# Autobot37/weatherforecastingtoolkit

Measured on AMD Instinct MI355X. Metric: SEVIR 384x384 frames/sec (AE train step), higher is better.
Workload: dtype f32; 1 GPU; experiments/ae_v2 conv AE (ae_64x8x8_lin.PosAwareAE_TF, img_size=384), 1x384x384 synthetic SEVIR frames, batch 32/GPU, fp32, fwd + L1 + bwd + AdamW + cosine-warmup LR; batch_per_gpu=32, global_batch=32, img_size=384, parallelism=dp1, params=215033281

## Files before the change

### include/wfae.h

```cpp
#ifndef WFAE_H
#define WFAE_H

#include <stddef.h>
#include <stdint.h>

#ifdef __cplusplus
extern "C" {
#endif

typedef void* wfae_stream_t;

typedef enum {
  WFAE_OK = 0,
  WFAE_ERR_BAD_SHAPE = -1,
  WFAE_ERR_NULL_POINTER = -2,
  WFAE_ERR_WORKSPACE = -3,
  WFAE_ERR_LAUNCH = -4,
  WFAE_ERR_UNSUPPORTED = -5
} wfae_status;

int wfae_version(void);
const char* wfae_last_error_string(void);
size_t wfae_workspace_bytes(int64_t max_weight_elems);

enum { WFAE_PRECISION_FP32 = 0, WFAE_PRECISION_BF16 = 1 };
int wfae_set_matmul_precision(int mode);
int wfae_get_matmul_precision(void);

int wfae_set_split_gemm(int on);
int wfae_get_split_gemm(void);

int wfae_set_c1n(int on);
int wfae_get_c1n(void);

int wfae_conv1x1_fwd(const float* x, const float* w, const float* bias, const float* res,
                     int64_t res_img_stride, float* y, int NB, int Cin, int Cout, int HW,
                     wfae_stream_t stream);
int wfae_conv1x1_fwd_stats(const float* x, const float* w, const float* bias, const float* res,
                           int64_t res_img_stride, float* y, int NB, int Cin, int Cout, int HW,
                           double* stat_part, int64_t stat_capacity, int* stat_rows, wfae_stream_t stream);
int wfae_conv1x1_fwd_bnact(const float* x, const float* bn_scale, const float* bn_shift, const float* w,
                           const float* bias, const float* res, int64_t res_img_stride, float* y, int NB, int Cin,
                           int Cout, int HW, double* stat_part, int64_t stat_capacity, int* stat_rows,
                           wfae_stream_t stream);
int wfae_conv1x1_bwd_weight_bnact(const float* dy, const float* x, const float* bn_scale, const float* bn_shift,
                                  float* dw, int NB, int Cin, int Cout, int HW, int accumulate, void* ws,
                                  size_t ws_bytes, wfae_stream_t stream);
int wfae_conv1x1_bwd_data(const float* dy, const float* w, float* dx, int NB, int Cin, int Cout,
                          int HW, wfae_stream_t stream);
int wfae_conv1x1_bwd_weight(const float* dy, const float* x, float* dw, int NB, int Cin, int Cout,
                            int HW, int accumulate, void* ws, size_t ws_bytes, wfae_stream_t stream);

int wfae_c1r_supported(int M, int K, int HW);
int wfae_c1r_stat_rows(int M, int K, int NB, int HW);
int wfae_c1r_fwd(const float* w, int64_t w_sm, int64_t w_sk, const float* x, const float* pro_scale, const float* pro_shift,
                 const float* res, float* y, int NB, int K, int M, int HW, double* stat_part, int64_t stat_capacity,
                 int* stat_rows, wfae_stream_t stream);
int wfae_c1r_bnred_supported(int M, int K, int HW);
int wfae_c1r_bnred(const float* w, int64_t w_sm, int64_t w_sk, const float* dt, const float* x, const float* bn_scale,
                   const float* bn_shift, const float* save_mean, const float* save_invstd, float* da, int NB, int K, int M, int HW,
                   double* part, int64_t part_capacity, int* part_rows, wfae_stream_t stream);
int wfae_bn_act_bwd_from_rows(const double* part, int rows, int C, float* dgamma, float* dbeta, int accumulate, void* ws,
                              size_t ws_bytes, wfae_stream_t stream);
int wfae_c1r_bndx(const float* w, int64_t w_sm, int64_t w_sk, const float* dt, const float* x, const float* gamma,
                  const float* bn_scale, const float* bn_shift, const float* save_mean, const float* save_invstd, const float* coef,
                  const float* res, float* dx, int NB, int K, int M, int HW, int training, wfae_stream_t stream);
int wfae_c1rb_supported(int M, int K, int HW);
int wfae_c1rb_stat_rows(int M, int K, int NB, int HW);
int wfae_c1rb_fwd(const float* w, int64_t w_sm, int64_t w_sk, const uint16_t* x, const float* pro_scale, const float* pro_shift,
                  const uint16_t* res, uint16_t* y, int NB, int K, int M, int HW, double* stat_part, int64_t stat_capacity,
                  int* stat_rows, wfae_stream_t stream);
int wfae_c1w_supported(int Cin, int Cout, int HW);
int wfae_c1w_bwd_weight(const float* dy, const float* x, const float* bn_scale, const float* bn_shift, float* dw, int NB, int Cin,
                        int Cout, int HW, int accumulate, void* ws, size_t ws_bytes, wfae_stream_t stream);
int wfae_c1w_bwd_weight_bf16(const uint16_t* dy, const uint16_t* x, const float* bn_scale, const float* bn_shift, float* dw, int NB,
                             int Cin, int Cout, int HW, int accumulate, void* ws, size_t ws_bytes, wfae_stream_t stream);
int wfae_linear_fwd(const float* x, const float* w, const float* bias, float* y, int B, int In,
                    int Out, void* ws, size_t ws_bytes, wfae_stream_t stream);
int wfae_linear_bwd_data(const float* dy, const float* w, float* dx, int B, int In, int Out,
                         wfae_stream_t stream);
int wfae_linear_bwd_weight(const float* dy, const float* x, float* dw, int B, int In, int Out,
                           int accumulate, wfae_stream_t stream);
int wfae_linear_bwd_data_splitk(const float* dy, const float* w, float* dx, int B, int In, int Out, void* ws,
                                size_t ws_bytes, wfae_stream_t stream);
int wfae_linear_bwd_weight_splitk(const float* dy, const float* x, float* dw, int B, int In, int Out, int accumulate,
                                  void* ws, size_t ws_bytes, wfae_stream_t stream);

int wfae_conv4x4s2_down(const float* hi, const float* w, float* lo, int NB, int Chi, int Clo,
                        int Hlo, int Wlo, wfae_stream_t stream);
int wfae_conv4x4s2_up(const float* lo, const float* w, float* hi, int NB, int Chi, int Clo, int Hlo,
                      int Wlo, void* ws, size_t ws_bytes, wfae_stream_t stream);
int wfae_conv4x4s2_wgrad(const float* lo, const float* hi, float* dw, int NB, int Chi, int Clo,
                         int Hlo, int Wlo, int accumulate, void* ws, size_t ws_bytes,
                         wfae_stream_t stream);

int wfae_dconv_fwd(const float* x, const float* w, const float* bias, float* y, int NB, int Cin,
                   int Cout, int H, int W, int KS, int stride, int pad, int groups,
                   wfae_stream_t stream);
int wfae_dconv_bwd_data(const float* dy, const float* w, float* dx, int NB, int Cin, int Cout,
                        int H, int W, int KS, int pad, int groups, wfae_stream_t stream);
int wfae_dconv_bwd_weight(const float* dy, const float* x, float* dw, int NB, int Cin, int Cout,
                          int H, int W, int KS, int stride, int pad, int groups, int accumulate,
                          void* ws, size_t ws_bytes, wfae_stream_t stream);

int wfae_gconv3x3_fwd(const float* x, const float* w, float* y, int NB, int C, int H, int W, int groups,
                      int transposed, void* ws, size_t ws_bytes, wfae_stream_t stream);
int wfae_gconv3x3_bwd_weight(const float* dy, const float* x, float* dw, int NB, int C, int H, int W,
                             int groups, int accumulate, void* ws, size_t ws_bytes, wfae_stream_t stream);

int wfae_bn_stats_train(const float* x, int NB, int C, int HW, const float* gamma,
                        const float* beta, float eps, float momentum, float* running_mean,
                        float* running_var, float* save_mean, float* save_invstd, float* scale,
                        float* shift, void* ws, size_t ws_bytes, wfae_stream_t stream);
int wfae_bn_stats_from_rows(const double* stat_part, int rows, int NB, int C, int HW, const float* gamma,
                            const float* beta, float eps, float momentum, float* running_mean,
                            float* running_var, float* save_mean, float* save_invstd, float* scale,
                            float* shift, void* ws, size_t ws_bytes, wfae_stream_t stream);
int wfae_bn_fold_eval(const float* gamma, const float* beta, const float* running_mean,
                      const float* running_var, float eps, float* save_mean, float* save_invstd,
                      float* scale, float* shift, int C, wfae_stream_t stream);
int wfae_bn_act_fwd(const float* x, const float* scale, const float* shift, float* y, int NB, int C,
                    int HW, int act, wfae_stream_t stream);
int wfae_bn_act_fwd_stats(const float* x, const float* scale, const float* shift, float* y, int NB, int C, int HW, int act,
                          double* part, int64_t part_capacity, int* splits_out, wfae_stream_t stream);
int wfae_bn_stats_from_parts(const double* part, int splits, int NB, int C, int HW, const float* gamma, const float* beta,
                             float eps, float momentum, float* running_mean, float* running_var, float* save_mean,
                             float* save_invstd, float* scale, float* shift, wfae_stream_t stream);
int wfae_bn_act_bwd(const float* dy, const float* x, const float* gamma, const float* scale,
                    const float* shift, const float* save_mean, const float* save_invstd,
// ... 304 lines not shown
```

### weatherforecastingtoolkit_amd/csrc/c1w.hip

```cpp
#include "common.h"

using namespace wfae;

namespace {

typedef float f32x16 __attribute__((ext_vector_type(16)));
typedef __bf16 bf16x8 __attribute__((ext_vector_type(8)));
typedef unsigned u32x4 __attribute__((ext_vector_type(4)));
typedef unsigned u32x2 __attribute__((ext_vector_type(2)));

struct C1WP {
  const void* P;
  const void* Q;
  float* slab;
  const float* pro_scale;
  const float* pro_shift;
  int MP, MQ, HW;
  int cpi;
  int kc;
  int ptiles;
};

constexpr int WNT = 512, WBK = 32;

// ... 182 lines not shown

  float* __restrict__ Cb = p.slab + (long)blockIdx.y * p.MP * p.MQ;
#pragma unroll
  for (int i = 0; i < TM; ++i)
#pragma unroll
    for (int j = 0; j < TN; ++j) {
      const int col = n0 + wn0 + 32 * j + r31;
#pragma unroll
      for (int q = 0; q < 16; ++q) {
        const int row = m0 + wm0 + 32 * i + (q & 3) + 8 * (q >> 2) + 4 * lh;
        if (row < p.MP && col < p.MQ) Cb[(long)row * p.MQ + col] = acc[i][j][q];
      }
    }
}

inline bool al16(const void* q) { return (reinterpret_cast<uintptr_t>(q) & 15) == 0; }

template <typename T, int PRO>
int launch_c1w(C1WP& p, int NB, hipStream_t st, const char* what) {
  const int tm = p.MP > 128 ? 2 : 1, tn = p.MQ > 64 ? 2 : 1;
  const int bm = 128 * tm, bn = 64 * tn;
  p.ptiles = cdiv(p.MP, bm);
  const int qtiles = cdiv(p.MQ, bn);
  const dim3 grid((unsigned)(p.ptiles * qtiles), (unsigned)(NB * p.cpi)), block(WNT);
  if (tm == 2 && tn == 2) hipLaunchKernelGGL((c1w_kernel<T, 2, 2, PRO>), grid, block, 0, st, p);
  else if (tm == 2) hipLaunchKernelGGL((c1w_kernel<T, 2, 1, PRO>), grid, block, 0, st, p);
  else if (tn == 2) hipLaunchKernelGGL((c1w_kernel<T, 1, 2, PRO>), grid, block, 0, st, p);
  else hipLaunchKernelGGL((c1w_kernel<T, 1, 1, PRO>), grid, block, 0, st, p);
  return check_launch(what);
}

inline bool c1w_shape_ok(int Cin, int Cout, int HW) {
  return HW % 32 == 0 && Cin % 32 == 0 && Cout % 32 == 0 && Cin >= 32 && Cout >= 32;
}

template <typename T>
int c1w_impl(const T* dy, const T* x, const float* bn_scale, const float* bn_shift, float* dw, int NB, int Cin, int Cout, int HW,
             int accumulate, void* ws, size_t ws_bytes, hipStream_t st, const char* what) {
  WFAE_REQUIRE(dy && x && dw && ws, WFAE_ERR_NULL_POINTER, "%s: null pointer", what);
  WFAE_REQUIRE(NB > 0 && Cin > 0 && Cout > 0 && HW > 0 && NB <= 65535, WFAE_ERR_BAD_SHAPE, "%s: bad shape", what);
  WFAE_REQUIRE(c1w_shape_ok(Cin, Cout, HW) && al16(dy) && al16(x), WFAE_ERR_UNSUPPORTED,
               "%s: needs HW %% 32 == 0, channel counts %% 32 == 0, 16-byte aligned tensors (Cin %d, Cout %d, HW %d)", what, Cin,
               Cout, HW);
  const bool x_is_p = Cin >= Cout;
  C1WP p = {};
  p.P = x_is_p ? (const void*)x : (const void*)dy;
  p.Q = x_is_p ? (const void*)dy : (const void*)x;
  p.MP = x_is_p ? Cin : Cout;
  p.MQ = x_is_p ? Cout : Cin;
  p.HW = HW;
  p.pro_scale = bn_scale;
  p.pro_shift = bn_shift;
  const size_t slab = (size_t)Cin * Cout * sizeof(float);
  const int tiles = cdiv(p.MP, p.MP > 128 ? 256 : 128) * cdiv(p.MQ, p.MQ > 64 ? 128 : 64);
  int cpi = cdiv(1024, (long)tiles * NB);
  const int max_cpi = HW / 256 > 0 ? HW / 256 : 1;
  if (cpi > max_cpi) cpi = max_cpi;
  if (cpi < 1) cpi = 1;
  while (cpi > 1 && (size_t)NB * cpi * slab > ws_bytes) --cpi;
  WFAE_REQUIRE((size_t)NB * cpi * slab <= ws_bytes, WFAE_ERR_WORKSPACE, "%s: workspace %zu < %zu", what, ws_bytes, (size_t)NB * slab);
  p.cpi = cpi;
  p.kc = cdiv(cdiv(HW, cpi), WBK) * WBK;
  p.cpi = cdiv(HW, p.kc);
  p.slab = (float*)ws;
  int rc;
  const int pro = bn_scale ? (x_is_p ? 1 : 2) : 0;
  if (pro == 0) rc = launch_c1w<T, 0>(p, NB, st, what);
  else if (pro == 1) rc = launch_c1w<T, 1>(p, NB, st, what);
  else rc = launch_c1w<T, 2>(p, NB, st, what);
  if (rc) return rc;
  return slab_reduce((const float*)ws, dw, nullptr, (long)Cin * Cout, p.MQ, NB * p.cpi, accumulate, st, x_is_p ? p.MP : 0);
}

}

extern "C" {

int wfae_c1w_supported(int Cin, int Cout, int HW) { return c1w_shape_ok(Cin, Cout, HW) ? 1 : 0; }

int wfae_c1w_bwd_weight(const float* dy, const float* x, const float* bn_scale, const float* bn_shift, float* dw, int NB, int Cin,
                        int Cout, int HW, int accumulate, void* ws, size_t ws_bytes, wfae_stream_t stream) {
  WFAE_REQUIRE((bn_scale != nullptr) == (bn_shift != nullptr), WFAE_ERR_NULL_POINTER, "c1w_bwd_weight: scale / shift go together");
  return c1w_impl(dy, x, bn_scale, bn_shift, dw, NB, Cin, Cout, HW, accumulate, ws, ws_bytes, (hipStream_t)stream, "c1w_bwd_weight");
}

int wfae_c1w_bwd_weight_bf16(const uint16_t* dy, const uint16_t* x, const float* bn_scale, const float* bn_shift, float* dw, int NB,
                             int Cin, int Cout, int HW, int accumulate, void* ws, size_t ws_bytes, wfae_stream_t stream) {
  WFAE_REQUIRE((bn_scale != nullptr) == (bn_shift != nullptr), WFAE_ERR_NULL_POINTER, "c1w_bwd_weight_bf16: scale / shift go together");
  return c1w_impl(dy, x, bn_scale, bn_shift, dw, NB, Cin, Cout, HW, accumulate, ws, ws_bytes, (hipStream_t)stream,
                  "c1w_bwd_weight_bf16");
}

}
```

### weatherforecastingtoolkit_amd/csrc/common.h

```cpp
#pragma once
#include <hip/hip_runtime.h>
#include <stdint.h>
#include <stdio.h>
#include <stdarg.h>
#include "../../include/wfae.h"

namespace wfae {

char* err_buf();
int fail(int code, const char* fmt, ...);
int matmul_precision();
bool split_gemm_enabled();

inline int check_launch(const char* what) {
  hipError_t e = hipGetLastError();
  if (e != hipSuccess) return fail(WFAE_ERR_LAUNCH, "%s: %s", what, hipGetErrorString(e));
  return WFAE_OK;
}

#define WFAE_REQUIRE(cond, code, ...) \
  do {                                \
    if (!(cond)) return ::wfae::fail(code, __VA_ARGS__); \
  } while (0)

// ... 157 lines not shown
__device__ __forceinline__ void st2(bf16_t* p, float2 v) { *reinterpret_cast<unsigned*>(p) = pack_bf16(v.x, v.y); }
__device__ __forceinline__ float rounded_as(const float*, float v) { return v; }
__device__ __forceinline__ float rounded_as(const bf16_t*, float v) { return bf16_lo(pack_bf16(v, 0.f)); }
__device__ __forceinline__ void st4(float* p, float4 v) { *reinterpret_cast<float4*>(p) = v; }
__device__ __forceinline__ void st4(bf16_t* p, float4 v) {
  *reinterpret_cast<uint2*>(p) = make_uint2(pack_bf16(v.x, v.y), pack_bf16(v.z, v.w));
}

__device__ __forceinline__ int aug_src_pixel(int i, int j, int H, int W, float c, float s, bool hflip, bool vflip) {
  const float cx = 0.5f * (float)W - 0.5f, cy = 0.5f * (float)H - 0.5f;
  const float xo = (float)j - cx, yo = (float)i - cy;
  const float xr = rintf(c * xo - s * yo + cx);
  const float yr = rintf(s * xo + c * yo + cy);
  if (!(xr >= 0.f && xr <= (float)(W - 1) && yr >= 0.f && yr <= (float)(H - 1))) return -1;
  int xs = (int)xr, ys = (int)yr;
  if (hflip) xs = W - 1 - xs;
  if (vflip) ys = H - 1 - ys;
  return ys * W + xs;
}

int c1_wgrad_mfma(int flip, const float* big, const float* small, float* dw, int NB, int C, int H, int W, int accumulate,
                  void* ws, size_t ws_bytes, hipStream_t st);
int c1_wgrad_mfma(int flip, const unsigned short* big, const float* small, float* dw, int NB, int C, int H, int W, int accumulate,
                  void* ws, size_t ws_bytes, hipStream_t st);
int c1conv3_wgrad(const float* dy, const float* x, float* dw, int NB, int C, int H, int W, int accumulate, void* ws,
                  size_t ws_bytes, hipStream_t st);

int wino_in(int variant, const float* hi, float* V, int NB, int Chi, int Hlo, int Wlo, hipStream_t st);
int wino_in_t(int variant, const float* dV, float* hi, int NB, int Chi, int Hlo, int Wlo, hipStream_t st);
int wino_out(int variant, const float* M, float* lo, int NB, int Clo, int Hlo, int Wlo, hipStream_t st);
int wino_out_t(int variant, const float* lo, float* Mt, int NB, int Clo, int Hlo, int Wlo, hipStream_t st);
int wino_out_stats(int variant, const float* M, float* lo, int NB, int Clo, int Hlo, int Wlo, double* part, hipStream_t st);
int wino_out_stat_splits(int variant, int NB, int Hlo, int Wlo);
int wino_in_t_stats(int variant, const float* dV, float* hi, int NB, int Chi, int Hlo, int Wlo, double* part, hipStream_t st);
int wino_weights(int variant, const float* w, float* U, int Clo, int Chi, hipStream_t st);
int wino_in_split(int variant, const float* hi, unsigned short* V3, int planes, int NB, int Chi, int Hlo, int Wlo, hipStream_t st);
int wino_out_t_split(int variant, const float* lo, unsigned short* Mt3, int planes, int NB, int Clo, int Hlo, int Wlo, hipStream_t st);
int wino_in_split(int variant, const unsigned short* hi, unsigned short* V3, int planes, int NB, int Chi, int Hlo, int Wlo, hipStream_t st);
int wino_out_t_split(int variant, const unsigned short* lo, unsigned short* Mt3, int planes, int NB, int Clo, int Hlo, int Wlo, hipStream_t st);
int wino_in_t(int variant, const float* dV, unsigned short* hi, int NB, int Chi, int Hlo, int Wlo, hipStream_t st);
int wino_in_t_stats(int variant, const float* dV, unsigned short* hi, int NB, int Chi, int Hlo, int Wlo, double* part, hipStream_t st);
int wino_out(int variant, const float* M, unsigned short* lo, int NB, int Clo, int Hlo, int Wlo, hipStream_t st);
int wino_out_stats(int variant, const float* M, unsigned short* lo, int NB, int Clo, int Hlo, int Wlo, double* part, hipStream_t st);
int wino_weights_split(int variant, const float* w, unsigned short* U3, unsigned short* Ut3, int planes, int Clo, int Chi,
                       hipStream_t st);
int split_gemm(int kind, int planes, const unsigned short* A, const unsigned short* B, float* C, int M, int N, int K,
               long a_plane, long b_plane, long a_y, long b_y, long c_y, int batches, int k_per_split, int splits,
               long c_split, hipStream_t st, const char* what);
int wino_weights_t(int variant, const float* dU, float* dw, int Clo, int Chi, int beta, hipStream_t st);

int c1n_launch(const float* w, bool transposed, const float* x, const float* scale, const float* shift, float* y, int NB, int K, int M,
               int HW, double* stat_part, int64_t stat_capacity, int* stat_rows, hipStream_t st, const char* what);

int slab_reduce(const float* slab, float* out, const float* bias_n, long MN, int N, int splits, int beta,
                hipStream_t st, int transpose_m = 0);

int gconv3_wgrad_valu(const float* dy, const float* x, float* dw, int NB, int C, int H, int W, int groups,
                      int accumulate, void* ws, size_t ws_bytes, hipStream_t st);
int gconv3_wgrad_mfma(const float* dy, const float* x, float* dw, int NB, int C, int H, int W, int groups,
                      int accumulate, void* ws, size_t ws_bytes, hipStream_t st);
int gconv3_wgrad_mfma(const unsigned short* dy, const unsigned short* x, float* dw, int NB, int C, int H, int W, int groups,
                      int accumulate, void* ws, size_t ws_bytes, hipStream_t st);

}
```

### weatherforecastingtoolkit_amd/functional.py

```python
from __future__ import annotations

import os

import torch
from torch.autograd import Function

from . import ops

BN_EPS = 1e-5


_overlap = False
_side = {}


STAT_FUSION = os.environ.get("WFAE_STAT_FUSION", "1") == "1"


FUSE_A1 = os.environ.get("WFAE_FUSE_A1", "1") == "1"
FUSE_A1_MAXC = 1 << 30
FUSE_A3 = os.environ.get("WFAE_FUSE_A3", "1") == "1"
FUSE_A3_MAXC = int(os.environ.get("WFAE_FUSE_A3_MAXC", "128"))
FUSE_A3_MAXC_C1R = max(FUSE_A3_MAXC, 256)


PRODUCER_STATS = os.environ.get("WFAE_PRODUCER_STATS", "1") == "1"


def set_wgrad_overlap(flag: bool):
    global _overlap
    _overlap = bool(flag)


def _side_stream():
    dev = torch.cuda.current_device()
    s = _side.get(dev)
    if s is None:
        s = _side[dev] = torch.cuda.Stream(device=dev)
    return s


_keep = []
_keep_bytes = [0]
_KEEP_LIMIT = 24 << 30


def join_side_stream():
    if _side:
        dev = torch.cuda.current_device()
        if dev in _side:
            torch.cuda.current_stream().wait_stream(_side[dev])
    _keep.clear()
    _keep_bytes[0] = 0


def _wgrad(fn, *tensors):
    if not _overlap:
        return fn()
    if _force_main[0]:
        _force_main[0] = False
        join_side_stream()
        return fn()
    side = _side_stream()
    side.wait_stream(torch.cuda.current_stream())
    with torch.cuda.stream(side):
        fn()
    _keep.extend(tensors)
    _keep_bytes[0] += sum(t.numel() * t.element_size() for t in tensors)
    if _keep_bytes[0] > _KEEP_LIMIT:
        join_side_stream()


_arena_grads = [True]


class detached_grads:

    def __enter__(self):
        self.prev = _arena_grads[0]
        _arena_grads[0] = False

    def __exit__(self, *exc):
        _arena_grads[0] = self.prev


_force_main = [False]


def grad_buffer(p):
    task = torch._C._current_graph_task_id()
    again = task >= 0 and getattr(p, "_wfae_lent_task", None) == task
    p._wfae_lent_task = task
    if p.grad is not None or again:
        _force_main[0] = True
        return torch.empty_like(p)
    v = getattr(p, "_wfae_grad_view", None)
    if v is not None and _arena_grads[0]:
        return v.view(v.shape)
    return torch.empty_like(p)


def _bn_stats(x, bn, training):
    if training:
        st = ops.bn_stats_train(x, bn.weight, bn.bias, bn.running_mean, bn.running_var, bn.eps, bn.momentum)
        bn._nbt_pending += 1
        return st
    return ops.bn_fold_eval(bn.weight, bn.bias, bn.running_mean, bn.running_var, bn.eps)


def _bn_stats_rows(sr, x, bn, training):
    if training and isinstance(sr, ops.StatParts):
        st = ops.bn_stats_from_parts(sr, tuple(x.shape), bn.weight, bn.bias, bn.running_mean, bn.running_var, bn.eps,
                                     bn.momentum)
        bn._nbt_pending += 1
        return st
    if training and sr is not None:
        st = ops.bn_stats_from_rows(sr, tuple(x.shape), bn.weight, bn.bias, bn.running_mean, bn.running_var, bn.eps,
                                    bn.momentum)
        bn._nbt_pending += 1
        return st
    return _bn_stats(x, bn, training)


# ... 361 lines not shown
class BottleneckFn(Function):
    @staticmethod
    def forward(ctx, x, g1, b1, w1, g2, b2, wg, g3, b3, w3, mod, x_stats=None):
        xc = _c(x)
        if xc is not x:
            x_stats = None
        x = xc
        bn1, bn2, bn3 = mod.f[0], mod.f[3], mod.f[6]
        groups = mod.f[5].groups
        training = _use_batch_stats(bn1)
        fuse = training and STAT_FUSION
        emit = fuse and getattr(mod, "emit_stats", False)
        C, mid, hw = x.shape[1], w1.shape[0], x.shape[2] * x.shape[3]
        sto = _storage(x)

        def route(op, m, k, pro=False, res="none"):
            return ops.conv1x1_route(op, m, k, hw, sto, pro, False, res)
        fused1 = FUSE_A1 and C <= FUSE_A1_MAXC and ops.conv1x1_bnact_supported(x, mid)
        r1, r3 = route("fwd", mid, C, fused1), route("fwd", C, mid, True, "ordinary")
        fused3 = (FUSE_A3 and C <= (FUSE_A3_MAXC_C1R if r3 in ("c1r", "c1rb") else FUSE_A3_MAXC)
                  and ops.conv1x1_bnact_supported((x.shape[0], mid) + x.shape[2:], C))
        if not fused3:
            r3 = route("fwd", C, mid, False, "ordinary")
        d1, d3 = (route("dgrad", C, mid), route("dgrad", mid, C)) if sto == "bf16" else (None, None)
        W1p, W3p = (ops.c1b_weights(w1), ops.c1b_weights(w3)) if "c1b" in (r1, r3, d1, d3) else ((None, None), (None, None))
        st1 = _bn_stats_rows(x_stats if (fuse or isinstance(x_stats, ops.StatParts)) else None, x, bn1, training)
        a1 = None if fused1 else ops.bn_act_fwd(x, st1, 1)
        t1, sr2 = _c1(w1, W1p[0], False, *((x, st1) if fused1 else (a1, None)), None, fuse, r1)
        st2 = _bn_stats_rows(sr2, t1, bn2, training)
        a2 = ops.bn_act_fwd(t1, st2, 1)
        t2 = _g3_fwd(a2, wg, groups)
        st3 = _bn_stats(t2, bn3, training)
        a3 = None if fused3 else ops.bn_act_fwd(t2, st3, 1)
        y, mod._out_stats = _c1(w3, W3p[0], False, *((t2, st3) if fused3 else (a3, None)), x, emit, r3)
        ctx.save_for_backward(x, _opt(a1), t1, a2, t2, _opt(a3), g1, w1, g2, wg, g3, w3,
                              st1.mean, st1.invstd, st1.scale, st1.shift,
                              st2.mean, st2.invstd, st2.scale, st2.shift,
                              st3.mean, st3.invstd, st3.scale, st3.shift,
                              _opt(W1p[1] if d1 == "c1b" else None), _opt(W3p[1] if d3 == "c1b" else None))
        ctx.training = training
        ctx.groups = groups
        ctx.betas = (b1, b2, b3)
        return y

    @staticmethod
    def backward(ctx, dy):
        (x, a1, t1, a2, t2, a3, g1, w1, g2, wg, g3, w3, *s) = ctx.saved_tensors
        st1, st2, st3 = _mk_stats(*s[0:4]), _mk_stats(*s[4:8]), _mk_stats(*s[8:12])
        W1t, W3t = s[12], s[13]
        tr = ctx.training
        dy = _c(dy)
        mid = w1.shape[0]
        dw3 = grad_buffer(w3)
        if a3.numel() == 0:
            _wgrad(lambda: ops.conv1x1_bwd_weight_bnact(dy, t2, st3, dw3), dy, t2, st3.scale, st3.shift)
        else:
            _wgrad(lambda: ops.conv1x1_bwd_weight(dy, a3, dw3), dy, a3)
        dg3, db3 = grad_buffer(g3), grad_buffer(ctx.betas[2])
        dt2 = _dgrad_bn(dy, w3, W3t, t2, g3, st3, dg3, db3, None, tr)
        dwg = grad_buffer(wg)
        _wgrad(lambda: _g3_wgrad(dt2, a2, dwg, ctx.groups), dt2, a2)
        da2 = _g3_dgrad(dt2, wg, mid, ctx.groups)
        del dt2
        dg2, db2 = grad_buffer(g2), grad_buffer(ctx.betas[1])
        dt1 = ops.bn_act_bwd(da2, t1, g2, st2, dg2, db2, None, 1, tr)
        del da2
        dw1 = grad_buffer(w1)
        if a1.numel() == 0:
            _wgrad(lambda: ops.conv1x1_bwd_weight_bnact(dt1, x, st1, dw1), dt1, x, st1.scale, st1.shift)
        else:
            _wgrad(lambda: ops.conv1x1_bwd_weight(dt1, a1, dw1), dt1, a1)
        dg1, db1 = grad_buffer(g1), grad_buffer(ctx.betas[0])
        dx = _dgrad_bn(dt1, w1, W1t, x, g1, st1, dg1, db1, dy, tr)
        return dx, dg1, db1, dw1, dg2, db2, dwg, dg3, db3, dw3, None, None


class Conv1x1Fn(Function):

    @staticmethod
    def forward(ctx, x, w, bias, pos):
        ctx.x_dtype = x.dtype
        x = ops.to_f32(_c(x))
        y = ops.conv1x1_fwd(x, w, bias, None if pos is None else _c(pos), pos is not None)
        ctx.save_for_backward(x, w)
        ctx.bias, ctx.pos = bias, pos
        return y

    @staticmethod
    def backward(ctx, dy):
        x, w = ctx.saved_tensors
        dy = ops.to_f32(_c(dy))
        nb, cout, h, wd = dy.shape
        dw = grad_buffer(w)
        ops.conv1x1_bwd_weight(dy, x, dw)
        dx = ops.to_dtype(ops.conv1x1_bwd_data(dy, w), ctx.x_dtype) if ctx.needs_input_grad[0] else None
        dbias = dpos = None
        if ctx.bias is not None:
            dbias = grad_buffer(ctx.bias)
            ops.reduce_sum(dy, nb, cout, h * wd, dbias)
        if ctx.pos is not None:
            dpos = grad_buffer(ctx.pos)
            ops.reduce_sum(dy, nb, cout * h * wd, 1, dpos)
        return dx, dw, dbias, dpos


def conv1x1(x, w, bias=None, pos=None):
    return Conv1x1Fn.apply(x, w, bias, pos)


class LinearFn(Function):
    @staticmethod
    def forward(ctx, x, w, bias):
# ... 803 lines not shown
```

### weatherforecastingtoolkit_amd/ops.py

```python
from __future__ import annotations

import ctypes
import os

import torch

from . import _lib

_WS_DEFAULT = int(os.environ.get("WFAE_WORKSPACE_MB", "512")) << 20
_ws = {}


def _stream():
    return torch.cuda.current_stream().cuda_stream


_prof = None


def profile_start():
    global _prof
    _prof = {}


# ... 154 lines not shown
def to_dtype(x, dtype):
    return to_bf16(x) if dtype == BF16 else to_f32(x)


def _p(t):
    return None if t is None else t.data_ptr()


class StatRows:
    __slots__ = ("part", "rows")

    def __init__(self, part, rows):
        self.part, self.rows = part, rows


class StatParts:
    __slots__ = ("part", "splits")

    def __init__(self, part, splits):
        self.part, self.splits = part, splits


def _rows_out(n, device):
    part = torch.empty(n, dtype=torch.float64, device=device)
    count = ctypes.c_int(0)
    return part, count, (part.data_ptr(), n, ctypes.cast(ctypes.pointer(count), ctypes.c_void_p))


_NO_ROWS = (None, 0, None)


_C1R = _C1R_BNRED = _C1R_BNDX = _C1RB = _C1B = _C1W = True


def set_c1r(on):
    global _C1R
    _C1R = bool(on)


def set_c1r_bnred(on):
    global _C1R_BNRED
    _C1R_BNRED = bool(on)


def set_c1r_bndx(on):
    global _C1R_BNDX
    _C1R_BNDX = bool(on)


def set_c1n(on):
    _lib.call("wfae_set_c1n", int(bool(on)))


def set_c1rb(on):
    global _C1RB
    _C1RB = bool(on)


def set_c1b(on):
    global _C1B
    _C1B = bool(on)


def set_c1w(on):
    global _C1W
    _C1W = bool(on)


def c1r_bndx_on():
    return _C1R_BNDX


def c1n_enabled():
    return bool(_lib.load().wfae_get_c1n())


def _precision():
    return _lib.load().wfae_get_matmul_precision()


def c1r_supported(m, k, hw):
    return _C1R and _SPLIT_GEMM and _precision() == 0 and bool(_lib.load().wfae_c1r_supported(int(m), int(k), int(hw)))


def c1r_bnred_supported(m, k, hw):
    return (_C1R and _C1R_BNRED and _SPLIT_GEMM and _precision() == 0
            and bool(_lib.load().wfae_c1r_bnred_supported(int(m), int(k), int(hw))))


def c1rb_supported(m, k, hw):
    return _C1RB and _precision() == 1 and bool(_lib.load().wfae_c1rb_supported(int(m), int(k), int(hw)))


def c1b_supported(m, k, hw):
    return _C1B and _precision() == 1 and bool(_lib.load().wfae_c1b_supported(int(m), int(k), int(hw)))


def conv1x1_bnact_supported(x, cout):
    nb, cin, h, wd = getattr(x, "shape", x)
    swapped = cin < cout and cin < 128
    return (h * wd) % 4 == 0 and h * wd >= 16 and cin % 4 == 0 and (cout % 4 == 0 or not swapped)


def conv1x1_route(op, m, k, hw, storage="f32", prologue=False, bias=False, residual="none"):
    if op == "wgrad":
        ok = _C1W and _lib.load().wfae_c1w_supported(int(k), int(m), int(hw))
        return "c1w" if ok and (_precision() == 1 if storage == "bf16" else (_precision() == 0 and _SPLIT_GEMM)) else "gemm"
    if bias or residual == "broadcast" or (residual == "ordinary" and m <= k):
        return "gemm"
    if storage == "f32":
        return "c1r" if c1r_supported(m, k, hw) else "gemm"
    rb = c1rb_supported(m, k, hw)
    if rb and not (prologue and m < k and k >= 256):
        return "c1rb"
    return "c1b" if (rb or c1b_supported(m, k, hw)) else "gemm"


def conv1x1_dgrad_bn_route(m, k, hw, storage="f32"):
    if storage == "f32" and c1r_bnred_supported(m, k, hw):
        return "bndx" if _C1R_BNDX else "bnred"
    return None


_C1_PEAK = {"c1r": PEAK_BF16_MFMA / 6, "c1rb": PEAK_BF16_MFMA, "c1b": PEAK_BF16_MFMA, "gemm": None}


def _c1_launch(fam, w, transposed, x, st=None, bias=None, res=None, res_broadcast=False, stats=False, label=None):
# ... 75 lines not shown
def conv1x1_bwd_data(dy, w):
    nb, cout, h, wd = dy.shape
    fam = "gemm" if dy.dtype == BF16 else conv1x1_route("dgrad", w.shape[1], cout, h * wd)
    return _c1_launch(fam, w, True, dy)[0]


def c1rb_fwd(w, transposed, x, st=None, res=None, stats=False, label="wfae_c1b_fwd"):
    r = _c1_launch("c1rb", w, transposed, x, st, None, res, False, stats, label)
    return r if stats else r[0]


def c1b_weights(w):
    _chk(w)
    cout, cin = w.shape[0], w.shape[1]
    Wb = torch.empty((cout, cin), dtype=BF16, device=w.device)
    Wtb = torch.empty((cin, cout), dtype=BF16, device=w.device)
    _call("wfae_c1b_weights", 0, 8 * w.numel(), _p(w), _p(Wb), _p(Wtb), cout, cin, _stream())
    return Wb, Wtb


def c1b_fwd(Wb, x, st=None, res=None, stats=False, label="wfae_c1b_fwd"):
    r = _c1_launch("c1b", Wb, False, x, st, None, res, False, stats, label)
    return r if stats else r[0]


def _c1_wgrad(dy, x, st, dw, accumulate):
    sfx, es = _chka(dy, x)
    _chk(dw)
    nb, cout, h, wd = dy.shape
    cin, n = x.shape[1], nb * h * wd
    pro = (None, None) if st is None else (_p(st.scale), _p(st.shift))
    peak = None
    if conv1x1_route("wgrad", cout, cin, h * wd, "bf16" if sfx else "f32", st is not None) == "c1w":
        name, peak = "wfae_c1w_bwd_weight" + sfx, PEAK_BF16_MFMA / (1 if sfx else 6)
    elif sfx:
        name = "wfae_conv1x1_bwd_weight_bf16"
    else:
        name, pro = ("wfae_conv1x1_bwd_weight", ()) if st is None else ("wfae_conv1x1_bwd_weight_bnact", pro)
    ws = workspace()
    _call(name, 2 * n * cin * cout, es * n * (cin + cout) + 4 * cin * cout, _p(dy), _p(x), *pro, _p(dw), nb, cin, cout, h * wd,
          int(accumulate), ws.data_ptr(), ws.numel(), _stream(), peak=peak,
          label="wfae_conv1x1_bwd_weight" if st is None else "wfae_conv1x1_bwd_weight_bnact")
    return dw


def conv1x1_bwd_weight(dy, x, dw, accumulate=False):
    return _c1_wgrad(dy, x, None, dw, accumulate)


def conv1x1_bwd_weight_bnact(dy, x, st, dw, accumulate=False):
    return _c1_wgrad(dy, x, st, dw, accumulate)


def c1r_bnred(w, dt, x, st, store=True):
    _chk(w, dt, x)
    nb, k, h, wd = dt.shape
    m, n = w.shape[1], nb * h * wd
    da = torch.empty((nb, m, h, wd), dtype=torch.float32, device=dt.device) if store else None
    part, rows, out = _rows_out(2 * int(_lib.load().wfae_c1r_stat_rows(m, k, nb, h * wd)) * m, dt.device)
    _call("wfae_c1r_bnred", 2 * n * k * m, 4 * (n * (k + (2 if store else 1) * m) + k * m), _p(w), 1, m, _p(dt), _p(x), _p(st.scale),
          _p(st.shift), _p(st.mean), _p(st.invstd), _p(da), nb, k, m, h * wd, *out, _stream(), label="wfae_conv1x1_bwd_data",
          peak=_C1_PEAK["c1r"])
    return da, StatRows(part[:2 * rows.value * m], rows.value)


def bn_act_bwd_from_rows(sr, c, dgamma, dbeta, accumulate=False):
    _chk(dgamma, dbeta)
    ws = workspace()
    _call("wfae_bn_act_bwd_from_rows", 0, 8 * sr.part.numel(), sr.part.data_ptr(), sr.rows, c, _p(dgamma), _p(dbeta), int(accumulate),
          ws.data_ptr(), ws.numel(), _stream(), label="wfae_bn_act_bwd[reduce]")
    return ws


def bn_act_bwd_dx(dy, x, gamma, st, res=None, act=1, training=True):
    _chk(dy, x, gamma, res)
    nb, c, h, wd = x.shape
    dx = torch.empty_like(x)
    ws = workspace()
    _call("wfae_bn_act_bwd", 0, 4 * x.numel() * (4 if res is not None else 3), _p(dy), _p(x), _p(gamma), _p(st.scale), _p(st.shift),
          _p(st.mean), _p(st.invstd), _p(res), _p(dx), None, None, nb, c, h * wd, act, int(training), 0, 2, ws.data_ptr(),
          ws.numel(), _stream(), label="wfae_bn_act_bwd[dx]")
    return dx


def c1r_bndx(w, dt, x, gamma, st, res=None, training=True):
    _chk(w, dt, x, gamma, res)
    nb, k, h, wd = dt.shape
    m, n = w.shape[1], nb * h * wd
    dx = torch.empty((nb, m, h, wd), dtype=torch.float32, device=dt.device)
    ws = workspace()
    _call("wfae_c1r_bndx", 2 * n * k * m, 4 * (n * (k + (3 if res is not None else 2) * m) + k * m), _p(w), 1, m, _p(dt), _p(x), _p(gamma),
          _p(st.scale), _p(st.shift), _p(st.mean), _p(st.invstd), ws.data_ptr(), _p(res), _p(dx), nb, k, m, h * wd, int(training),
          _stream(), label="wfae_c1r_bndx", peak=_C1_PEAK["c1r"])
    return dx


def linear_fwd(x, w, bias=None):
    _chk(x, w, bias)
    b, inf = x.shape
    out = w.shape[0]
    y = torch.empty((b, out), dtype=x.dtype, device=x.device)
    ws = workspace()
    _call("wfae_linear_fwd", 2 * b * inf * out, 4 * (inf * out + b * (inf + out)), _p(x), _p(w), _p(bias), _p(y), b, inf, out, ws.data_ptr(), ws.numel(), _stream())
    return y


# ... 1586 lines not shown
```

Baseline: 178.4 frames/s.

## Fuse 1x1 conv weight-grad and data-grad into one kernel sharing dy tiles

Adds a c1wd kernel for the last 1x1 conv of bottleneck blocks (C=128/256, mid=C/4). It computes dW3 (dy x gelu(bn(t2))) and da3 (W3^T x dy) in one pass, using split-bf16 MFMA, so dy is read from memory once instead of twice. The dgrad is then fed into the BN-act backward, replacing the separate dgrad path. In exchange it runs on the main stream rather than overlapping wgrad on the side stream, and it adds register and LDS pressure.

```diff
diff --git a/include/wfae.h b/include/wfae.h
--- a/include/wfae.h
+++ b/include/wfae.h
@@ -75,6 +75,11 @@
                         int Cout, int HW, int accumulate, void* ws, size_t ws_bytes, wfae_stream_t stream);
 int wfae_c1w_bwd_weight_bf16(const uint16_t* dy, const uint16_t* x, const float* bn_scale, const float* bn_shift, float* dw, int NB,
                              int Cin, int Cout, int HW, int accumulate, void* ws, size_t ws_bytes, wfae_stream_t stream);
+int wfae_set_c1wd(int on);
+int wfae_get_c1wd(void);
+int wfae_c1wd_supported(int C, int mid, int HW);
+int wfae_c1wd_bwd(const float* dy, const float* t2, const float* bn_scale, const float* bn_shift, const float* w3, float* dw3,
+                  float* da3, int NB, int C, int mid, int HW, int accumulate, void* ws, size_t ws_bytes, wfae_stream_t stream);
 int wfae_linear_fwd(const float* x, const float* w, const float* bias, float* y, int B, int In,
                     int Out, void* ws, size_t ws_bytes, wfae_stream_t stream);
 int wfae_linear_bwd_data(const float* dy, const float* w, float* dx, int B, int In, int Out,
diff --git a/weatherforecastingtoolkit_amd/csrc/c1w.hip b/weatherforecastingtoolkit_amd/csrc/c1w.hip
--- a/weatherforecastingtoolkit_amd/csrc/c1w.hip
+++ b/weatherforecastingtoolkit_amd/csrc/c1w.hip
@@ -258,16 +258,8 @@
   p.pro_scale = bn_scale;
   p.pro_shift = bn_shift;
   const size_t slab = (size_t)Cin * Cout * sizeof(float);
-  const int tiles = cdiv(p.MP, p.MP > 128 ? 256 : 128) * cdiv(p.MQ, p.MQ > 64 ? 128 : 64);
-  int cpi = cdiv(1024, (long)tiles * NB);
-  const int max_cpi = HW / 256 > 0 ? HW / 256 : 1;
-  if (cpi > max_cpi) cpi = max_cpi;
-  if (cpi < 1) cpi = 1;
-  while (cpi > 1 && (size_t)NB * cpi * slab > ws_bytes) --cpi;
-  WFAE_REQUIRE((size_t)NB * cpi * slab <= ws_bytes, WFAE_ERR_WORKSPACE, "%s: workspace %zu < %zu", what, ws_bytes, (size_t)NB * slab);
-  p.cpi = cpi;
-  p.kc = cdiv(cdiv(HW, cpi), WBK) * WBK;
-  p.cpi = cdiv(HW, p.kc);
+  WFAE_REQUIRE(c1w_chunks(p.MP, p.MQ, NB, HW, ws_bytes, &p.cpi, &p.kc), WFAE_ERR_WORKSPACE, "%s: workspace %zu < %zu", what, ws_bytes,
+               (size_t)NB * slab);
   p.slab = (float*)ws;
   int rc;
   const int pro = bn_scale ? (x_is_p ? 1 : 2) : 0;
@@ -280,6 +272,24 @@
 
 }
 
+namespace wfae {
+
+bool c1w_chunks(int MP, int MQ, int NB, int HW, size_t ws_bytes, int* cpi_out, int* kc_out) {
+  const size_t slab = (size_t)MP * MQ * sizeof(float);
+  const int tiles = cdiv(MP, MP > 128 ? 256 : 128) * cdiv(MQ, MQ > 64 ? 128 : 64);
+  int cpi = cdiv(1024, (long)tiles * NB);
+  const int max_cpi = HW / 256 > 0 ? HW / 256 : 1;
+  if (cpi > max_cpi) cpi = max_cpi;
+  if (cpi < 1) cpi = 1;
+  while (cpi > 1 && (size_t)NB * cpi * slab > ws_bytes) --cpi;
+  if ((size_t)NB * cpi * slab > ws_bytes) return false;
+  *kc_out = cdiv(cdiv(HW, cpi), WBK) * WBK;
+  *cpi_out = cdiv(HW, *kc_out);
+  return true;
+}
+
+}
+
 extern "C" {
 
 int wfae_c1w_supported(int Cin, int Cout, int HW) { return c1w_shape_ok(Cin, Cout, HW) ? 1 : 0; }
diff --git a/weatherforecastingtoolkit_amd/csrc/c1wd.hip b/weatherforecastingtoolkit_amd/csrc/c1wd.hip
--- /dev/null
+++ b/weatherforecastingtoolkit_amd/csrc/c1wd.hip
@@ -0,0 +1,304 @@
+#include "common.h"
+#include <atomic>
+#include <stdlib.h>
+#include <type_traits>
+
+using namespace wfae;
+
+namespace {
+
+typedef float f32x4 __attribute__((ext_vector_type(4)));
+typedef float f32x16 __attribute__((ext_vector_type(16)));
+typedef __bf16 bf16x8 __attribute__((ext_vector_type(8)));
+typedef short s16x4 __attribute__((ext_vector_type(4)));
+typedef short s16x8 __attribute__((ext_vector_type(8)));
+typedef unsigned u32x4 __attribute__((ext_vector_type(4)));
+typedef unsigned u32x2 __attribute__((ext_vector_type(2)));
+
+struct C1WDP {
+  const float* dy;
+  const float* t2;
+  const float* w3;
+  const float* pro_scale;
+  const float* pro_shift;
+  float* slab;
+  float* da;
+  int HW;
+  int cpi;
+  int kc;
+};
+
+constexpr int DNT = 512, DBK = 32;
+
+__device__ __forceinline__ unsigned off_row(int r, int c) { return (unsigned)(r * 64 + ((c ^ ((r >> 2) & 3)) << 4)); }
+
+__device__ __forceinline__ void split_pair(float a, float b, unsigned& h, unsigned& m, unsigned& l) {
+  h = pack_bf16(a, b);
+  const float ra = a - bf16_lo(h), rb = b - bf16_hi(h);
+  m = pack_bf16(ra, rb);
+  l = pack_bf16(ra - bf16_lo(m), rb - bf16_hi(m));
+}
+
+template <int C>
+__global__ __launch_bounds__(DNT, C == 128 ? 4 : 2) void c1wd_kernel(C1WDP p) {
+  constexpr int M = C / 4;
+  constexpr int TM = C / 128;
+  constexpr int WQ = M / 32;
+  constexpr int NDW = 4 * WQ;
+  constexpr bool BOTH = NDW == 8;
+  constexpr int KCH = C / 32;
+  constexpr int LPR = 8;
+  constexpr int P_LD = C * LPR, Q_LD = M * LPR;
+  constexpr int P_IT = P_LD / DNT;
+  static_assert(P_LD % DNT == 0 && Q_LD <= DNT, "loader");
+  constexpr int A_PLANE_B = C * 64, B_PLANE_B = M * 64;
+  constexpr int A_STAGE_B = 3 * A_PLANE_B, STAGE_B = 3 * (A_PLANE_B + B_PLANE_B);
+  __shared__ __attribute__((aligned(16))) unsigned char smem[2 * STAGE_B];
+  const int t = threadIdx.x, lane = t & 63;
+  const int wave = __builtin_amdgcn_readfirstlane(t >> 6);
+  const int img = blockIdx.x / p.cpi, chunk = blockIdx.x - img * p.cpi;
+  const int k_begin = chunk * p.kc;
+  const int k_end = min(p.HW, k_begin + p.kc);
+  const int nsteps = (k_end - k_begin) / DBK;
+  const bool do_dw = BOTH || wave < NDW, do_da = BOTH || wave >= NDW;
+
+  const float* Pb = p.dy + (long)img * C * p.HW + k_begin;
+  const float* Qb = p.t2 + (long)img * M * p.HW + k_begin;
+  const float* p_src[P_IT];
+  unsigned p_dst[P_IT];
+#pragma unroll
+  for (int j = 0; j < P_IT; ++j) {
+    const int idx = t + j * DNT, r = idx / LPR, e = idx % LPR;
+    p_src[j] = Pb + (long)r * p.HW + e * 4;
+    p_dst[j] = off_row(r, e >> 1) + (unsigned)((e & 1) * 8);
+  }
+  const bool q_on = Q_LD == DNT || t < Q_LD;
+  const int q_r = q_on ? t / LPR : 0, q_e = t % LPR;
+  const float* q_src = Qb + (long)q_r * p.HW + q_e * 4;
+  const unsigned q_dst = off_row(q_r, q_e >> 1) + (unsigned)((q_e & 1) * 8);
+  const float q_s = p.pro_scale[q_r], q_h = p.pro_shift[q_r];
+  u32x4 rp[P_IT], rq;
+  auto load_global = [&]() {
+#pragma unroll
+    for (int j = 0; j < P_IT; ++j) rp[j] = *reinterpret_cast<const u32x4*>(p_src[j]);
+    if (q_on) rq = *reinterpret_cast<const u32x4*>(q_src);
+  };
+  auto advance = [&](bool more) {
+#pragma unroll
+    for (int j = 0; j < P_IT; ++j) p_src[j] += more ? DBK : 0;
+    q_src += more ? DBK : 0;
+  };
+  auto put = [&](unsigned char* base, int plane_b, unsigned dst, u32x4 r, bool act, float s, float h) {
+    const unsigned u0 = r[0], u1 = r[1], u2 = r[2], u3 = r[3];
+    float v0 = __uint_as_float(u0), v1 = __uint_as_float(u1), v2 = __uint_as_float(u2), v3 = __uint_as_float(u3);
+    if (act) {
+      v0 = gelu_f(fmaf(v0, s, h)); v1 = gelu_f(fmaf(v1, s, h));
+      v2 = gelu_f(fmaf(v2, s, h)); v3 = gelu_f(fmaf(v3, s, h));
+    }
+    unsigned h0, m0, l0, h1, m1, l1;
+    split_pair(v0, v1, h0, m0, l0);
+    split_pair(v2, v3, h1, m1, l1);
+    *reinterpret_cast<u32x2*>(base + dst) = u32x2{h0, h1};
+    *reinterpret_cast<u32x2*>(base + plane_b + dst) = u32x2{m0, m1};
+    *reinterpret_cast<u32x2*>(base + 2 * plane_b + dst) = u32x2{l0, l1};
+  };
+  auto store_lds = [&](int buf) {
+    unsigned char* s = smem + buf * STAGE_B;
+#pragma unroll
+    for (int j = 0; j < P_IT; ++j) put(s, A_PLANE_B, p_dst[j], rp[j], false, 0.f, 0.f);
+    if (q_on) put(s + A_STAGE_B, B_PLANE_B, q_dst, rq, true, q_s, q_h);
+  };
+
+  const int wm0 = (BOTH ? (wave >> 1) : (wave & 3)) * (32 * TM), wn0 = BOTH ? (wave & 1) * 32 : 0;
+  const int r31 = lane & 31, lh = lane >> 5;
+  const unsigned a_rd = (unsigned)((wm0 + r31) * 64), b_rd = (unsigned)((wn0 + r31) * 64);
+  const int a_x = (r31 >> 2) & 3;
+  f32x16 acc[TM];
+  struct Frag {
+    bf16x8 a[TM][3], b[3];
+  };
+  auto read_frag = [&](Frag& f, int buf, int ks) {
+    const unsigned char* s = smem + buf * STAGE_B;
+    const unsigned a_c = (unsigned)(((2 * ks + lh) ^ a_x) << 4);
+#pragma unroll
+    for (int i = 0; i < TM; ++i)
+#pragma unroll
+      for (int pl = 0; pl < 3; ++pl)
+        f.a[i][pl] = *reinterpret_cast<const bf16x8*>(s + pl * A_PLANE_B + a_rd + i * (32 * 64) + a_c);
+#pragma unroll
+    for (int pl = 0; pl < 3; ++pl) f.b[pl] = *reinterpret_cast<const bf16x8*>(s + A_STAGE_B + pl * B_PLANE_B + b_rd + a_c);
+  };
+  auto mfma_frag = [&](const Frag& f) {
+#pragma unroll
+    for (int i = 0; i < TM; ++i) {
+      f32x16 c = acc[i];
+      c = __builtin_amdgcn_mfma_f32_32x32x16_bf16(f.a[i][2], f.b[0], c, 0, 0, 0);
+      c = __builtin_amdgcn_mfma_f32_32x32x16_bf16(f.a[i][0], f.b[2], c, 0, 0, 0);
+      c = __builtin_amdgcn_mfma_f32_32x32x16_bf16(f.a[i][1], f.b[1], c, 0, 0, 0);
+      c = __builtin_amdgcn_mfma_f32_32x32x16_bf16(f.a[i][1], f.b[0], c, 0, 0, 0);
+      c = __builtin_amdgcn_mfma_f32_32x32x16_bf16(f.a[i][0], f.b[1], c, 0, 0, 0);
+      c = __builtin_amdgcn_mfma_f32_32x32x16_bf16(f.a[i][0], f.b[0], c, 0, 0, 0);
+      acc[i] = c;
+    }
+  };
+
+  const int dtile = BOTH ? wave : (wave & 3);
+  const int mt = dtile >> 1, pt = dtile & 1;
+  const int n16 = lane & 15, kg = lane >> 4, tq = n16 >> 2, tp = n16 & 3;
+  bf16x8 wa[KCH][3];
+  auto load_weights = [&]() {
+#pragma unroll
+    for (int ch = 0; ch < KCH; ++ch) {
+      const float* src = p.w3 + (long)(32 * ch + 8 * kg) * M + 16 * mt + n16;
+      float v[8];
+#pragma unroll
+      for (int e = 0; e < 8; ++e) v[e] = src[e * M];
+      u32x4 h, m, l;
+#pragma unroll
+      for (int e = 0; e < 4; ++e) {
+        unsigned qh, qm, ql;
+        split_pair(v[2 * e], v[2 * e + 1], qh, qm, ql);
+        h[e] = qh; m[e] = qm; l[e] = ql;
+      }
+      wa[ch][0] = __builtin_bit_cast(bf16x8, h);
+      wa[ch][1] = __builtin_bit_cast(bf16x8, m);
+      wa[ch][2] = __builtin_bit_cast(bf16x8, l);
+    }
+  };
+  unsigned tr_rd[2];
+#pragma unroll
+  for (int hf = 0; hf < 2; ++hf) tr_rd[hf] = off_row(8 * kg + 4 * hf + tq, 2 * pt + (tp >> 1)) + 8u * (unsigned)(tp & 1);
+  float* const da_dst = p.da + ((long)img * M + 16 * mt + 4 * kg) * p.HW + k_begin + 16 * pt + n16;
+  auto da_step = [&](int buf, int st) {
+    const unsigned char* s = smem + buf * STAGE_B;
+    constexpr int PA[6] = {2, 0, 1, 1, 0, 0}, PB[6] = {0, 2, 1, 0, 1, 0};
+    f32x4 d = {0.f, 0.f, 0.f, 0.f};
+#pragma unroll
+    for (int ch = 0; ch < KCH; ++ch) {
+      bf16x8 b[3];
+#pragma unroll
+      for (int pl = 0; pl < 3; ++pl) {
+        s16x4 part[2];
+#pragma unroll
+        for (int hf = 0; hf < 2; ++hf)
+          part[hf] = __builtin_amdgcn_ds_read_tr16_b64_v4i16(
+              (s16x4 __attribute__((address_space(3)))*)(s + pl * A_PLANE_B + ch * (32 * 64) + tr_rd[hf]));
+        b[pl] = __builtin_bit_cast(bf16x8, __builtin_shufflevector(part[0], part[1], 0, 1, 2, 3, 4, 5, 6, 7));
+      }
+#pragma unroll
+      for (int pr = 0; pr < 6; ++pr) d = __builtin_amdgcn_mfma_f32_16x16x32_bf16(wa[ch][PA[pr]], b[PB[pr]], d, 0, 0, 0);
+    }
+    float* o = da_dst + 32 * st;
+#pragma unroll
+    for (int q = 0; q < 4; ++q) o[(long)q * p.HW] = d[q];
+  };
+
+  auto run = [&](auto dwc, auto dac) {
+    constexpr bool DW = decltype(dwc)::value, DA = decltype(dac)::value;
+    if constexpr (DW) {
+#pragma unroll
+      for (int i = 0; i < TM; ++i)
+#pragma unroll
+        for (int q = 0; q < 16; ++q) acc[i][q] = 0.f;
+    }
+    if constexpr (DA) load_weights();
+    if (nsteps > 0) {
+      Frag f0, f1;
+      load_global();
+      advance(nsteps > 1);
+      store_lds(0);
+      load_global();
+      advance(nsteps > 2);
+      __syncthreads();
+      if constexpr (DW) read_frag(f0, 0, 0);
+      for (int st = 0; st < nsteps; ++st) {
+        const int cur = st & 1;
+        if constexpr (DW) read_frag(f1, cur, 1);
+        store_lds(cur ^ 1);
+        load_global();
+        advance(st + 3 < nsteps);
+        if constexpr (DW) mfma_frag(f0);
+        if constexpr (DA) da_step(cur, st);
+        __builtin_amdgcn_sched_barrier(0);
+        __syncthreads();
+        __builtin_amdgcn_sched_barrier(0);
+        if constexpr (DW) {
+          read_frag(f0, cur ^ 1, 0);
+          mfma_frag(f1);
+        }
+        __builtin_amdgcn_sched_barrier(0);
+      }
+    }
+    if constexpr (DW) {
+      float* __restrict__ Cb = p.slab + (long)blockIdx.x * C * M;
+#pragma unroll
+      for (int i = 0; i < TM; ++i)
+#pragma unroll
+        for (int q = 0; q < 16; ++q) {
+          const int row = wm0 + 32 * i + (q & 3) + 8 * (q >> 2) + 4 * lh;
+          Cb[(long)row * M + wn0 + r31] = acc[i][q];
+        }
+    }
+  };
+  if constexpr (BOTH) run(std::true_type{}, std::true_type{});
+  else if (do_dw) run(std::true_type{}, std::false_type{});
+  else run(std::false_type{}, std::true_type{});
+}
+
+std::atomic<int> g_c1wd{-1};
+inline bool c1wd_on() {
+  int v = g_c1wd.load(std::memory_order_relaxed);
+  if (v < 0) {
+    const char* e = getenv("WFAE_C1WD");
+    v = (e && e[0] == '0') ? 0 : 1;
+    g_c1wd.store(v, std::memory_order_relaxed);
+  }
+  return v == 1;
+}
+
+inline bool al16(const void* q) { return (reinterpret_cast<uintptr_t>(q) & 15) == 0; }
+
+inline bool c1wd_shape_ok(int C, int mid, int HW) { return (C == 128 || C == 256) && mid * 4 == C && HW > 0 && HW % 64 == 0; }
+
+}
+
+extern "C" {
+
+int wfae_set_c1wd(int on) {
+  g_c1wd.store(on ? 1 : 0, std::memory_order_relaxed);
+  return WFAE_OK;
+}
+
+int wfae_get_c1wd(void) { return c1wd_on() ? 1 : 0; }
+
+int wfae_c1wd_supported(int C, int mid, int HW) {
+  return (c1wd_on() && c1wd_shape_ok(C, mid, HW) && wfae::split_gemm_enabled()) ? 1 : 0;
+}
+
+int wfae_c1wd_bwd(const float* dy, const float* t2, const float* bn_scale, const float* bn_shift, const float* w3, float* dw3,
+                  float* da3, int NB, int C, int mid, int HW, int accumulate, void* ws, size_t ws_bytes, wfae_stream_t stream) {
+  WFAE_REQUIRE(dy && t2 && bn_scale && bn_shift && w3 && dw3 && da3 && ws, WFAE_ERR_NULL_POINTER, "c1wd_bwd: null pointer");
+  WFAE_REQUIRE(NB > 0 && C > 0 && mid > 0 && HW > 0 && NB <= 65535 && (int64_t)NB * HW < (1ll << 31), WFAE_ERR_BAD_SHAPE,
+               "c1wd_bwd: bad shape");
+  WFAE_REQUIRE(c1wd_shape_ok(C, mid, HW), WFAE_ERR_UNSUPPORTED,
+               "c1wd_bwd: serves C = 128 or 256 with mid = C / 4 and HW %% 64 == 0 (C %d, mid %d, HW %d)", C, mid, HW);
+  WFAE_REQUIRE(c1wd_on() && wfae::split_gemm_enabled(), WFAE_ERR_UNSUPPORTED,
+               "c1wd_bwd: needs fp32 precision with the split GEMMs on and wfae_set_c1wd(1)");
+  WFAE_REQUIRE(al16(dy) && al16(t2), WFAE_ERR_UNSUPPORTED, "c1wd_bwd: dy and t2 must be 16-byte aligned");
+  C1WDP p = {};
+  p.dy = dy; p.t2 = t2; p.w3 = w3;
+  p.pro_scale = bn_scale; p.pro_shift = bn_shift;
+  p.slab = (float*)ws; p.da = da3;
+  p.HW = HW;
+  WFAE_REQUIRE(c1w_chunks(C, mid, NB, HW, ws_bytes, &p.cpi, &p.kc), WFAE_ERR_WORKSPACE, "c1wd_bwd: workspace %zu < %zu", ws_bytes,
+               (size_t)NB * C * mid * sizeof(float));
+  hipStream_t st = (hipStream_t)stream;
+  const dim3 grid((unsigned)(NB * p.cpi)), block(DNT);
+  if (C == 128) hipLaunchKernelGGL((c1wd_kernel<128>), grid, block, 0, st, p);
+  else hipLaunchKernelGGL((c1wd_kernel<256>), grid, block, 0, st, p);
+  const int rc = check_launch("c1wd_bwd");
+  if (rc) return rc;
+  return slab_reduce((const float*)ws, dw3, nullptr, (long)C * mid, mid, NB * p.cpi, accumulate, st, 0);
+}
+
+}
diff --git a/weatherforecastingtoolkit_amd/csrc/common.h b/weatherforecastingtoolkit_amd/csrc/common.h
--- a/weatherforecastingtoolkit_amd/csrc/common.h
+++ b/weatherforecastingtoolkit_amd/csrc/common.h
@@ -233,6 +233,8 @@
 int c1n_launch(const float* w, bool transposed, const float* x, const float* scale, const float* shift, float* y, int NB, int K, int M,
                int HW, double* stat_part, int64_t stat_capacity, int* stat_rows, hipStream_t st, const char* what);
 
+bool c1w_chunks(int MP, int MQ, int NB, int HW, size_t ws_bytes, int* cpi_out, int* kc_out);
+
 int slab_reduce(const float* slab, float* out, const float* bias_n, long MN, int N, int splits, int beta,
                 hipStream_t st, int transpose_m = 0);
 
diff --git a/weatherforecastingtoolkit_amd/functional.py b/weatherforecastingtoolkit_amd/functional.py
--- a/weatherforecastingtoolkit_amd/functional.py
+++ b/weatherforecastingtoolkit_amd/functional.py
@@ -69,6 +69,14 @@
     _keep_bytes[0] += sum(t.numel() * t.element_size() for t in tensors)
     if _keep_bytes[0] > _KEEP_LIMIT:
         join_side_stream()
+
+
+def _on_main(fn):
+    if _force_main[0]:
+        _force_main[0] = False
+        if _overlap:
+            join_side_stream()
+    return fn()
 
 
 _arena_grads = [True]
@@ -536,12 +544,20 @@
         dy = _c(dy)
         mid = w1.shape[0]
         dw3 = grad_buffer(w3)
+        da3 = None
         if a3.numel() == 0:
-            _wgrad(lambda: ops.conv1x1_bwd_weight_bnact(dy, t2, st3, dw3), dy, t2, st3.scale, st3.shift)
+            if ops.conv1x1_wd_route(dy.shape[1], mid, dy.shape[2] * dy.shape[3], _storage(dy)) == "c1wd":
+                da3 = _on_main(lambda: ops.conv1x1_bwd_wd(dy, t2, st3, w3, dw3))
+            if da3 is None:
+                _wgrad(lambda: ops.conv1x1_bwd_weight_bnact(dy, t2, st3, dw3), dy, t2, st3.scale, st3.shift)
         else:
             _wgrad(lambda: ops.conv1x1_bwd_weight(dy, a3, dw3), dy, a3)
         dg3, db3 = grad_buffer(g3), grad_buffer(ctx.betas[2])
-        dt2 = _dgrad_bn(dy, w3, W3t, t2, g3, st3, dg3, db3, None, tr)
+        if da3 is not None:
+            dt2 = ops.bn_act_bwd(da3, t2, g3, st3, dg3, db3, None, 1, tr)
+        else:
+            dt2 = _dgrad_bn(dy, w3, W3t, t2, g3, st3, dg3, db3, None, tr)
+        del da3
         dwg = grad_buffer(wg)
         _wgrad(lambda: _g3_wgrad(dt2, a2, dwg, ctx.groups), dt2, a2)
         da2 = _g3_dgrad(dt2, wg, mid, ctx.groups)
diff --git a/weatherforecastingtoolkit_amd/ops.py b/weatherforecastingtoolkit_amd/ops.py
--- a/weatherforecastingtoolkit_amd/ops.py
+++ b/weatherforecastingtoolkit_amd/ops.py
@@ -230,6 +230,10 @@
     _lib.call("wfae_set_c1n", int(bool(on)))
 
 
+def set_c1wd(on):
+    _lib.call("wfae_set_c1wd", int(bool(on)))
+
+
 def set_c1rb(on):
     global _C1RB
     _C1RB = bool(on)
@@ -251,6 +255,10 @@
 
 def c1n_enabled():
     return bool(_lib.load().wfae_get_c1n())
+
+
+def c1wd_enabled():
+    return bool(_lib.load().wfae_get_c1wd())
 
 
 def _precision():
@@ -432,6 +440,39 @@
     return _c1_wgrad(dy, x, st, dw, accumulate)
 
 
+C1WD_MIN_HW = 512
+
+
+def conv1x1_wd_supported(c, mid, hw, storage="f32"):
+    return (storage == "f32" and _SPLIT_GEMM and _precision() == 0 and bool(_lib.load().wfae_c1wd_supported(int(c), int(mid), int(hw)))
+            and conv1x1_route("wgrad", c, mid, hw, "f32", True) == "c1w" and conv1x1_route("dgrad", mid, c, hw) == "c1r")
+
+
+def conv1x1_wd_route(c, mid, hw, storage="f32"):
+    return "c1wd" if hw >= C1WD_MIN_HW and conv1x1_wd_supported(c, mid, hw, storage) else "pair"
+
+
+def conv1x1_bwd_wd(dy, t2, st, w3, dw3, accumulate=False):
+    if st is None or dy.dtype != torch.float32 or t2.dtype != torch.float32:
+        return None
+    nb, c, h, wd = dy.shape
+    mid, hw = t2.shape[1], h * wd
+    if not conv1x1_wd_supported(c, mid, hw):
+        return None
+    _chk(dy, t2, w3, dw3)
+    if tuple(t2.shape) != (nb, mid, h, wd) or w3.numel() != c * mid or dw3.numel() != c * mid:
+        raise _lib.WfaeError("conv1x1_bwd_wd: dy (N, C, H, W), t2 (N, C/4, H, W), w3 and dw3 (C, C/4)")
+    if (dy.data_ptr() | t2.data_ptr()) & 15:
+        return None
+    da = torch.empty_like(t2)
+    n = nb * hw
+    ws = workspace()
+    _call("wfae_c1wd_bwd", 4 * n * c * mid, 4 * n * (c + 2 * mid) + 8 * c * mid, _p(dy), _p(t2), _p(st.scale), _p(st.shift), _p(w3),
+          _p(dw3), _p(da), nb, c, mid, hw, int(accumulate), ws.data_ptr(), ws.numel(), _stream(), peak=PEAK_BF16_MFMA / 6,
+          label="wfae_c1wd_bwd")
+    return da
+
+
 def c1r_bnred(w, dt, x, st, store=True):
     _chk(w, dt, x)
     nb, k, h, wd = dt.shape
```

Measured after the change: 181.0 frames/s, median of 6. +1.5%, better.
